# Cc19245/gaussian-splatting_CC-Comments

Hardware: AMD Instinct MI355X
Metric: train iters/sec (fwd+bwd rasterize) @1980x1080, 1M Gaussians (higher is better)
Workload: dtype f32; 1 GPU; C3: 1000000 Gaussians, SH deg 3, 1980x1080, mu=-5.0, seed 0; P=1000000, parallelism=single view

## Files before the change

gaussian-splatting_cc-comments_amd/csrc/api.hip:

```cpp
#include <stdarg.h>
#include <stdio.h>
#include <string.h>

#include <atomic>
#include <cmath>
#include <mutex>
#include <string>
#include <vector>

#include "gsr_internal.h"
#include "../../include/gsr_aa.h"
#include "../../include/gsr_contrib.h"
#include "../../include/gsr_features.h"
#include "../../include/gsr_distortion.h"
#include "../../include/gsr_median.h"
#include "../../include/gsr_normals.h"
#include "../../include/gsr_loss_ext.h"
#include "../../include/gsr_bilagrid.h"
#include "../../include/gsr_mcmc.h"
#include "../../include/gsr_densify.h"
#include "../../include/gsr_filter3d.h"
#include "../../include/gsr_knn.h"
#include "../../include/gsr_rigidity.h"

// ... 170 lines not shown
	o->col_table = off;      off = gsr_align_up(off + gsr_tilebin_col_table_bytes(n));
	o->rshape = off;         off = gsr_align_up(off + n * 8);
	o->total = off;
	return GSR_OK;
}

extern "C" int gsr_image_layout_of(int W, int H, gsr_image_layout* o)
{
	if (W < 0 || H < 0 || !o) return gsr_fail(GSR_ERR_INVALID_ARGUMENT, "gsr_image_layout_of: bad arguments");
	const size_t N = (size_t)W * H, T = (size_t)gsr_grid_x(W) * gsr_grid_y(H);
	size_t off = 0;
	o->final_C = off;          off = gsr_align_up(off + 3 * N * 4);
	o->final_T = off;          off = gsr_align_up(off + N * 4);
	o->n_contrib = off;        off = gsr_align_up(off + N * 4);
	o->ranges = off;           off = gsr_align_up(off + T * 8);
	o->tile_max_contrib = off; off = gsr_align_up(off + T * 4);
	{
		const size_t extra_f = 3 * (size_t)gsr_tile_order_max_split((int)T), extra_b = gsr_tile_order_max_segments((int)T);
		o->tile_order = off;   off = gsr_align_up(off + (T + (extra_f > extra_b ? extra_f : extra_b) + 1) * 4);
	}
	o->total = off;
	return GSR_OK;
}

extern "C" int gsr_binning_layout_of(int P, int64_t R, int W, int H, gsr_binning_layout* o)
{
	(void)P;
	if (R < 0 || W < 0 || H < 0 || !o) return gsr_fail(GSR_ERR_INVALID_ARGUMENT, "gsr_binning_layout_of: bad arguments");
	const size_t n = (size_t)R;
	size_t off = 0;
	o->point_list = off;     off = gsr_align_up(off + n * 4);
	o->point_list_alt = off; off = gsr_align_up(off + n * 4);
	o->tile_keys = off;      off = gsr_align_up(off + n * 4);
	o->tile_keys_alt = off;  off = gsr_align_up(off + n * 4);
	{
		const size_t a = gsr_radix_table_bytes(n), b = gsr_tilebin_row_table_bytes(n);
		o->sort_table = off; off = gsr_align_up(off + (a > b ? a : b));
	}
	o->checkpoints = off;    off = gsr_align_up(off + gsr_checkpoint_records(R) * 256 * sizeof(float4));
	o->total = off;
	o->tile_key_bytes = (size_t)gsr_tile_key_bytes(gsr_grid_x(W) * gsr_grid_y(H), n);
	o->column_pairs = gsr_tilebin_applies(W, H) ? 1 : 0;
	return GSR_OK;
}

extern "C" size_t gsr_geometry_bytes(int P)
{
	gsr_geometry_layout l;
	return gsr_geometry_layout_of(P, &l) == GSR_OK ? l.total : 0;
}
extern "C" size_t gsr_image_bytes(int W, int H)
{
	gsr_image_layout l;
	return gsr_image_layout_of(W, H, &l) == GSR_OK ? l.total : 0;
}
extern "C" size_t gsr_binning_bytes(int P, int64_t R, int W, int H)
{
	gsr_binning_layout l;
	return gsr_binning_layout_of(P, R, W, H, &l) == GSR_OK ? l.total : 0;
}
extern "C" size_t gsr_backward_scratch_bytes(int P, int64_t R)
{
	(void)P;
	if (R < 0) return 0;
	return gsr_align_up((size_t)R * sizeof(GsrGradSlot));
}
// ... 164 lines not shown
	g.sorted_block_sums = (uint32_t*)(b + l.scan_temp);
	g.block_tiles = (uint32_t*)(b + l.scan_temp + gsr_align_up(((size_t)P + GSR_PREPROCESS_BLOCK - 1) / GSR_PREPROCESS_BLOCK * 4));
	g.sort_table = (void*)(b + l.sort_table);
	g.col_table = (void*)(b + l.col_table);
	g.rshape = (uint2*)(b + l.rshape);
	return g;
}

GsrImage gsr_image_view(void* blob, int W, int H)
{
	gsr_image_layout l;
	gsr_image_layout_of(W, H, &l);
	char* b = (char*)blob;
	GsrImage im;
	im.final_C = (float*)(b + l.final_C);
	im.final_T = (float*)(b + l.final_T);
	im.n_contrib = (uint32_t*)(b + l.n_contrib);
	im.ranges = (uint2*)(b + l.ranges);
	im.tile_max_contrib = (uint32_t*)(b + l.tile_max_contrib);
	im.tile_order = (uint32_t*)(b + l.tile_order);
	return im;
}

GsrBinning gsr_binning_view(void* blob, int P, int64_t R, int W, int H)
{
	gsr_binning_layout l;
	gsr_binning_layout_of(P, R, W, H, &l);
	char* b = (char*)blob;
	GsrBinning bn;
	bn.point_list = (uint32_t*)(b + l.point_list);
	bn.point_list_alt = (uint32_t*)(b + l.point_list_alt);
	bn.tile_keys = (uint32_t*)(b + l.tile_keys);
	bn.tile_keys_alt = (uint32_t*)(b + l.tile_keys_alt);
	bn.sort_table = (void*)(b + l.sort_table);
	bn.checkpoints = (float4*)(b + l.checkpoints);
	return bn;
}

extern "C" uint32_t gsr_get_higher_msb(uint32_t n)
{
	uint32_t msb = sizeof(n) * 4;
	uint32_t step = msb;
	while (step > 1) {
		step /= 2;
		if (n >> msb) msb += step; else msb -= step;
	}
	if (n >> msb) msb++;
	return msb;
}

struct GsrThreadDevice {
	hipStream_t aux_stream = nullptr;
	hipEvent_t aux_fork = nullptr, aux_join = nullptr;
	uint32_t* status_host = nullptr;
	hipEvent_t status_event = nullptr;
	hipStream_t copy_stream = nullptr;
	hipEvent_t copy_fork = nullptr;
};
struct GsrThreadState { GsrThreadDevice dev[GSR_MAX_DEVICES]; };
static thread_local GsrThreadState g_thread;

extern "C" int gsr_thread_release(void)
{
	g_err[0] = 0;
	int rc = GSR_OK;
	for (int d = 0; d < GSR_MAX_DEVICES; d++) {
// ... 1338 lines not shown
```

gaussian-splatting_cc-comments_amd/csrc/gsr_internal.h:

```cpp
#pragma once
#include <hip/hip_runtime.h>
#include <hip/hip_ext.h>
#include <stddef.h>
#include <stdint.h>

#include <type_traits>

#include "../../include/gsr.h"
#include "../../include/gsr_aux.h"
#include "../../include/gsr_cam.h"
#include "../../include/gsr_absgrad.h"
#include "../../include/gsr_camera_model.h"
#include "../../include/gsr_cam_cm.h"
#include "gsr_device.h"

#define GSR_PREPROCESS_BLOCK 256
#define GSR_COUNT_PARTS 64
#define GSR_STATUS_NEGMIN (4 + GSR_COUNT_PARTS)
#define GSR_STATUS_MAX (4 + 2 * GSR_COUNT_PARTS)
#define GSR_STATUS_WORDS (4 + 3 * GSR_COUNT_PARTS)

#ifndef GSR_SLOT_COOP
#define GSR_SLOT_COOP 30
#endif
// ... 15 lines not shown
	uint8_t* clamped;
	float* sh_ddir;
	uint32_t* status;

	uint32_t* sorted_block_sums;
	uint32_t* block_tiles;
	void* sort_table;
	void* col_table;
};

#ifndef GSR_CKPT_STRIDE
#define GSR_CKPT_STRIDE 512
#endif
#ifndef GSR_SPLIT_MIN_LIST
#define GSR_SPLIT_MIN_LIST 640
#endif
#define GSR_CKPT_MAX_SEGMENTS 15
static inline size_t gsr_checkpoint_records(int64_t R) { return (size_t)(R / GSR_CKPT_STRIDE) + 2; }

struct GsrImage {
	float* final_C;
	float* final_T;
	uint32_t* n_contrib;
	uint2* ranges;
	uint32_t* tile_max_contrib;
	uint32_t* tile_order;
};

struct GsrBinning {
	uint32_t* point_list;
	uint32_t* point_list_alt;
	uint32_t* tile_keys;
	uint32_t* tile_keys_alt;
	void* sort_table;
	float4* checkpoints;
};

struct GsrAuxBlend {
	float* out_depth;
	float* out_alpha;
	float* ckpt_depth;
	float* final_D;
	const float* dL_ddepth;
	const float* dL_dalpha;
};

GsrGeometry gsr_geometry_view(void* blob, int P);
GsrImage gsr_image_view(void* blob, int W, int H);
GsrBinning gsr_binning_view(void* blob, int P, int64_t R, int W, int H);

struct GsrFrame {
	int P, W, H;
	int64_t R;
	GsrGeometry g;
	GsrImage img;
	GsrBinning bin;
	GsrGradSlot* slots;
	uint8_t* slot_valid;
	hipStream_t s;
	int debug;
	bool cull;
};

struct GsrCamTarget {
	float* rows;
	float* dL_dviewmatrix;
// ... 255 lines not shown
```

gaussian-splatting_cc-comments_amd/csrc/render_backward.hip:

```cpp
#include "render_common.h"
#include <type_traits>

#define GSR_BWD_NV 9
#ifndef GSR_BWD_BAND_LAST
#define GSR_BWD_BAND_LAST 1
#endif
#define GSR_BWD_FLUSH 4
typedef float v2f __attribute__((ext_vector_type(2)));

GSR_TILE_CLOCK_BUFFER(gsr_backward_tile_clock, gsr_debug_tile_clock_backward)

__device__ __forceinline__ float gsr_add_halves(v2f a)
{
	float r;
	asm("v_add_f32_e32 %0, %1, %2" : "=v"(r) : "v"(a.x), "v"(a.y));
	return r;
}

template <int M> struct gsr_half;
template <> struct gsr_half<3> {
	typedef v2f type;
	static __device__ __forceinline__ v2f get(const v2f& a) { return a; }
	static __device__ __forceinline__ void set(v2f& d, v2f s) { d = s; }
	static __device__ __forceinline__ v2f select(bool h0, bool h1, v2f a) { return v2f{h0 ? a.x : 0.f, h1 ? a.y : 0.f}; }
};
template <> struct gsr_half<1> {
	typedef float type;
	static __device__ __forceinline__ float get(const v2f& a) { return a.x; }
	static __device__ __forceinline__ void set(v2f& d, float s) { d.x = s; }
	static __device__ __forceinline__ float select(bool h0, bool, float a) { return h0 ? a : 0.f; }
};
template <> struct gsr_half<2> {
	typedef float type;
	static __device__ __forceinline__ float get(const v2f& a) { return a.y; }
	static __device__ __forceinline__ void set(v2f& d, float s) { d.y = s; }
	static __device__ __forceinline__ float select(bool, bool h1, float a) { return h1 ? a : 0.f; }
};
__device__ __forceinline__ float gsr_fma(float a, float b, float c) { return __builtin_fmaf(a, b, c); }
__device__ __forceinline__ v2f gsr_fma(v2f a, v2f b, v2f c) { return __builtin_elementwise_fma(a, b, c); }
__device__ __forceinline__ float gsr_exp2(float a) { return __builtin_amdgcn_exp2f(a); }
__device__ __forceinline__ v2f gsr_exp2(v2f a) { return v2f{__builtin_amdgcn_exp2f(a.x), __builtin_amdgcn_exp2f(a.y)}; }
__device__ __forceinline__ float gsr_rcp(float a) { return __builtin_amdgcn_rcpf(a); }
__device__ __forceinline__ v2f gsr_rcp(v2f a) { return v2f{__builtin_amdgcn_rcpf(a.x), __builtin_amdgcn_rcpf(a.y)}; }
__device__ __forceinline__ float gsr_min99(float a) { return fminf(0.99f, a); }
__device__ __forceinline__ v2f gsr_min99(v2f a) { return v2f{fminf(0.99f, a.x), fminf(0.99f, a.y)}; }
__device__ __forceinline__ float gsr_lo(float a) { return a; }
__device__ __forceinline__ float gsr_lo(v2f a) { return a.x; }
__device__ __forceinline__ float gsr_hi(float a) { return a; }
__device__ __forceinline__ float gsr_hi(v2f a) { return a.y; }
__device__ __forceinline__ float gsr_abs_sum(float a) { return __builtin_fabsf(a); }
__device__ __forceinline__ float gsr_abs_sum(v2f a) { return __builtin_fabsf(a.x) + __builtin_fabsf(a.y); }

template <bool AUX, bool ABS>
__global__ void __launch_bounds__(64 * GSR_WAVES_PER_WG) __attribute__((amdgpu_waves_per_eu((AUX && ABS) ? 3 : 4, 4))) gsr_render_backward_wave_kernel(
	int W, int H, int gx, int nslots, const uint2* __restrict__ ranges, const uint32_t* __restrict__ point_list,
	const GsrSplat* __restrict__ splat, const float4* __restrict__ checkpoints, const float* __restrict__ final_C, const uint32_t* __restrict__ slot_base, const float* __restrict__ bg,
	const float* __restrict__ final_Ts, const uint32_t* __restrict__ n_contrib, const uint32_t* __restrict__ tile_max_contrib,
	const uint32_t* __restrict__ tile_order, const float* __restrict__ dL_dpixels, GsrGradSlot* __restrict__ slots,
	uint8_t* __restrict__ slot_valid, int cull, GsrAuxBlend aux)
{
	__shared__ float4 s_rec[GSR_WAVES_PER_WG][AUX ? 6 : 5][64];
	__shared__ uint32_t s_bands[GSR_WAVES_PER_WG][64];
	__shared__ float s_red[GSR_WAVES_PER_WG][64 * 9 + 8];
	__shared__ __attribute__((aligned(16))) float s_pend[GSR_WAVES_PER_WG][(AUX || ABS) ? 4 : GSR_BWD_FLUSH * 128];
	constexpr bool ONE_BAND = !(AUX || ABS);
	const int wave = threadIdx.x >> 6, lane = threadIdx.x & 63;
	const int slot_id = blockIdx.x * GSR_WAVES_PER_WG + wave;
	if (slot_id >= nslots) return;
	GSR_TILE_CLOCK_START();
	GSR_TILE_STAT(unsigned long long st_staged = 0; unsigned long long st_pairs = 0; unsigned long long st_pairs_hit = 0; unsigned long long st_reductions = 0; unsigned long long st_lanes_hit = 0;
	              unsigned long long st_one_mask = 0; unsigned long long st_one_last = 0;)
	const uint32_t entry = __builtin_amdgcn_readfirstlane(tile_order[slot_id]);
	if (entry == 0xFFFFFFFFu) return;
	const int tile = (int)(entry & 0x0FFFFFFFu);
	const int seg1 = (int)(entry >> 28);
	float4(*rec)[64] = s_rec[wave];
	uint32_t* recb = s_bands[wave];

	const int tx = tile % gx, ty = tile / gx;
	const int px = tx * GSR_TILE_X + (lane & 15);
	const int py0 = ty * GSR_TILE_Y + (lane >> 4);
	const v2f pfx2 = {(float)px, (float)px};
	const float x0f = (float)(tx * GSR_TILE_X), y0f = (float)(ty * GSR_TILE_Y);

	const uint2 range = ranges[tile];
	const int n = (int)min(range.y - range.x, tile_max_contrib[tile]);
	int seg_a = 0, top = n;
	if (seg1) {
		const int coarse = (int)__builtin_amdgcn_readfirstlane(tile_order[nslots]);
		const int nblk = (n + GSR_CKPT_STRIDE - 1) / GSR_CKPT_STRIDE, m = (nblk + GSR_CKPT_MAX_SEGMENTS - 1) / GSR_CKPT_MAX_SEGMENTS * coarse;
		seg_a = (seg1 - 1) * m * GSR_CKPT_STRIDE;
		top = min(n, seg1 * m * GSR_CKPT_STRIDE);
	}
	const int nw = top - seg_a;
	const uint32_t* plist = point_list + range.x;
	const size_t plane = (size_t)H * W;
	const float bg0 = bg[0], bg1 = bg[1], bg2 = bg[2];
	const float ddelx_dx = 0.5f * W, ddely_dy = 0.5f * H;

	v2f T[2], tfb[2];
	v2f ac0[2], ac1[2], ac2[2];
	v2f dp0[2], dp1[2], dp2[2];
	v2f dpD[2], acD[2];
	int last_contributor[GSR_PIX_PER_LANE];
	v2f pfy[2];
#pragma unroll
	for (int k = 0; k < GSR_PIX_PER_LANE; k++) {
		const int py = py0 + 4 * k;
		const bool inside = px < W && py < H;
		const uint32_t pix_id = inside ? (uint32_t)(W * py + px) : 0u;
		const float Tf = inside ? final_Ts[pix_id] : 0.f;
		const float d0 = inside ? dL_dpixels[pix_id] : 0.f;
		const float d1 = inside ? dL_dpixels[plane + pix_id] : 0.f;
		const float d2 = inside ? dL_dpixels[2 * plane + pix_id] : 0.f;
		last_contributor[k] = inside ? (int)n_contrib[pix_id] : 0;
		T[k >> 1][k & 1] = Tf;
		dp0[k >> 1][k & 1] = d0; dp1[k >> 1][k & 1] = d1; dp2[k >> 1][k & 1] = d2;
		if (AUX) {
			const float dD = (inside && aux.dL_ddepth) ? aux.dL_ddepth[pix_id] : 0.f;
			const float dA = (inside && aux.dL_dalpha) ? aux.dL_dalpha[pix_id] : 0.f;
			dpD[k >> 1][k & 1] = dD;
			tfb[k >> 1][k & 1] = -Tf * ((bg0 * d0 + bg1 * d1 + bg2 * d2) - dA);
		} else {
			tfb[k >> 1][k & 1] = -Tf * (bg0 * d0 + bg1 * d1 + bg2 * d2);
		}
		pfy[k >> 1][k & 1] = (float)py;
	}
#pragma unroll
	for (int p = 0; p < 2; p++) {
		ac0[p] = ac1[p] = ac2[p] = v2f{0.f, 0.f};
		if (AUX) acD[p] = v2f{0.f, 0.f};
	}
	if (top < n) {
		const float4* ck = checkpoints + ((size_t)(range.x + (uint32_t)top) / GSR_CKPT_STRIDE) * 256 + lane;
#pragma unroll
		for (int k = 0; k < GSR_PIX_PER_LANE; k++) {
			const int py = py0 + 4 * k;
			const bool inside = px < W && py < H;
			const uint32_t pix_id = inside ? (uint32_t)(W * py + px) : 0u;
			if (inside && last_contributor[k] > top) {
				const float4 c = ck[64 * k];
				const float inv = 1.0f / c.x;
				T[k >> 1][k & 1] = c.x;
				ac0[k >> 1][k & 1] = (final_C[pix_id] - c.y) * inv;
				ac1[k >> 1][k & 1] = (final_C[plane + pix_id] - c.z) * inv;
				ac2[k >> 1][k & 1] = (final_C[2 * plane + pix_id] - c.w) * inv;
				if (AUX) acD[k >> 1][k & 1] = (aux.final_D[pix_id] - aux.ckpt_depth[((size_t)(range.x + (uint32_t)top) / GSR_CKPT_STRIDE) * 256 + lane + 64 * k]) * inv;
			}
		}
	}
	int band_last[GSR_PIX_PER_LANE];
#pragma unroll
	for (int k = 0; k < GSR_PIX_PER_LANE; k++) {
		int m = last_contributor[k];
#pragma unroll
		for (int off = 32; off > 0; off >>= 1) m = max(m, __shfl_xor(m, off, 64));
		band_last[k] = __builtin_amdgcn_readfirstlane(m);
	}

	float4 ra = make_float4(0, 0, 0, 0), rb = ra, rc = ra;
	uint32_t sbase = 0u;
	if (lane < nw) {
		const uint32_t id = plist[top - 1 - lane];
		const float4* p = reinterpret_cast<const float4*>(splat + id);
		ra = p[0]; rb = p[1]; rc = p[2];
		sbase = slot_base[id];
	}
	uint32_t id_next = (64 + lane < nw) ? plist[top - 1 - (64 + lane)] : 0u;
	const int out_index = lane >> 3;
	float* const red_w = s_red[wave] + lane * 9;
	const float* const red_r = s_red[wave] + (lane & 7) * 9 + (lane >> 3);
	constexpr int red_step = 72;
	const float out_scale = (out_index >= 2 && out_index <= 4) ? -0.5f : 1.0f;
	const float k01 = out_index == 0 ? -ddelx_dx : -ddely_dy;
	const int f_inst = (lane >> 3) & 3, f_val = lane & 7;
	float* const pend_w = s_pend[wave] + lane;
	const float* const pend_r = s_pend[wave] + f_inst * 128 + (lane >> 5) * 64 + f_val * 8;
	const float f_scale = (f_val >= 2 && f_val <= 4) ? -0.5f : 1.0f;
	const float f_k01 = f_val == 0 ? -ddelx_dx : -ddely_dy;
	const bool f_word = lane < 32 || f_val == 0;
	int npend = 0;
	uint32_t pend_j = 0u;

	for (int base = 0; base < nw; base += 64) {
		const uint32_t reach = (base + lane < nw) ? (cull ? gsr_tile_band_mask(ra.x, ra.y, ra.z, ra.w, rb.x, rb.y, x0f, y0f) : 0xFu) : 0u;
		const int position = top - 1 - (base + lane);
		uint32_t live = 0u;
#pragma unroll
		for (int k = 0; k < GSR_PIX_PER_LANE; k++) live |= position < band_last[k] ? 1u << k : 0u;
		if (!(cull && GSR_BWD_BAND_LAST)) live = ((live & 3u) ? 3u : 0u) | ((live & 12u) ? 12u : 0u);
		const uint32_t bands = reach & live;
		const bool keep = cull ? bands != 0u : reach != 0u;
		const unsigned long long mask = __builtin_amdgcn_ballot_w64(keep);
		const int cnt = __popcll(mask);
		GSR_TILE_STAT(st_staged += (unsigned)cnt;)
		if (keep) {
			const int pos = gsr_mbcnt(mask);
			const uint32_t rmin = __float_as_uint(rb.z), rwh = __float_as_uint(rb.w);
			const uint32_t slot = sbase + ((uint32_t)ty - (rmin >> 16)) * (rwh & 0xffffu) + ((uint32_t)tx - (rmin & 0xffffu));
			rec[0][pos] = make_float4(ra.x, ra.x, ra.y, ra.y);
			rec[1][pos] = make_float4(-0.5f * ra.z, -0.5f * ra.z, ra.w, ra.w);
			rec[2][pos] = make_float4(-0.5f * rb.x, -0.5f * rb.x, rb.y, rb.y);
			rec[3][pos] = make_float4(rc.x, rc.x, rc.y, rc.y);
			rec[4][pos] = make_float4(rc.z, rc.z, __int_as_float(position), __uint_as_float(slot));
			if (AUX) rec[5][pos] = make_float4(rc.w, rc.w, 0.f, 0.f);
			recb[pos] = bands | (reach << 4);
		}
		if (base + 64 + lane < nw) {
			const float4* p = reinterpret_cast<const float4*>(splat + id_next);
			ra = p[0]; rb = p[1]; rc = p[2];
			sbase = slot_base[id_next];
		}
		id_next = (base + 128 + lane < nw) ? plist[top - 1 - (base + 128 + lane)] : 0u;
		__builtin_amdgcn_wave_barrier();

#pragma clang loop unroll(disable)
		for (int j = 0; j < cnt; j++) {
			const float4 R0 = rec[0][j], R1 = rec[1][j], R2 = rec[2][j], R3 = rec[3][j], R4 = rec[4][j];
			const int contributor = __builtin_amdgcn_readfirstlane(__float_as_int(R4.z));
			const uint32_t bands = __builtin_amdgcn_readfirstlane(recb[j]);
			const v2f X = {R0.x, R0.y}, Y = {R0.z, R0.w}, CA = {R1.x, R1.y}, CB = {R1.z, R1.w}, CC = {R2.x, R2.y}, OP = {R2.z, R2.w};
			const v2f C0 = {R3.x, R3.y}, C1 = {R3.z, R3.w}, C2 = {R4.x, R4.y};
			v2f V = {0.f, 0.f};
			if (AUX) { const float4 R5 = rec[5][j]; V = v2f{R5.x, R5.y}; }
			const v2f dx = X - pfx2;
			const v2f ax2 = (CA * dx) * dx, bdx = CB * dx;
			v2f CBh = {0.f, 0.f};
			float absx = 0.f, absy = 0.f;
			if constexpr (ABS) CBh = -0.5f * CB;
			v2f acc[GSR_BWD_NV + 1];
#pragma unroll
			for (int i = 0; i < GSR_BWD_NV + 1; i++) acc[i] = v2f{-0.f, -0.f};
			unsigned long long any = 0ull;
			auto pair = [&](auto pc, auto mc) {
				constexpr int p = decltype(pc)::value, M = decltype(mc)::value;
				typedef gsr_half<M> Hf;
				typedef typename Hf::type V_t;
				const V_t dxh = Hf::get(dx);
				const V_t dy = Hf::get(Y) - Hf::get(pfy[p]);
				const V_t power = (Hf::get(ax2) + (Hf::get(CC) * dy) * dy) - Hf::get(bdx) * dy;
				const V_t pl = power * 1.44269504088896340736f;
				const V_t G = gsr_exp2(pl);
				const V_t og = Hf::get(OP) * G;
				const V_t araw = gsr_min99(og);
				bool hit0 = false, hit1 = false;
				unsigned long long hits = 0ull;
// ... 112 lines not shown
					pend_w[npend * 128] = tcol;
					pend_w[npend * 128 + 64] = v[8];
					pend_j |= (uint32_t)j << (8 * npend);
					npend++;
				}
			}
			if (!(AUX || ABS) && (npend == GSR_BWD_FLUSH || (npend != 0 && j == cnt - 1))) {
				__builtin_amdgcn_wave_barrier();
				const float4 q0 = *reinterpret_cast<const float4*>(pend_r), q1 = *reinterpret_cast<const float4*>(pend_r + 4);
				const uint32_t jf = (pend_j >> (8 * f_inst)) & 0xFFu;
				const float* const rj = reinterpret_cast<const float*>(&rec[0][jf]);
				const float ca = rj[4 * 64], cb = rj[4 * 64 + 2], cc = rj[8 * 64];
				const uint32_t slot = __float_as_uint(rj[16 * 64 + 3]);
				asm volatile("" ::"v"(q0.x), "v"(q1.x), "v"(ca), "v"(cb), "v"(cc), "v"(slot));
				const float t = ((q0.x + q0.y) + (q0.z + q0.w)) + ((q1.x + q1.y) + (q1.z + q1.w));
				const float t9 = gsr_sum8(t);
				const float other = gsr_dpp_mov<0xB1, 0xF, 0xF, true>(t);
				const float r01 = f_k01 * __builtin_fmaf(-2.0f, (f_val == 0 ? ca : cc) * t, cb * other);
				const float r = f_val < 2 ? r01 : f_scale * t;
				if (f_inst < npend) {
					if (f_word) reinterpret_cast<float*>(slots + slot)[lane < 32 ? f_val : 8] = lane < 32 ? r : t9;
					if (lane >= 32 && f_val == 0) slot_valid[slot] = 1;
				}
				npend = 0;
				pend_j = 0u;
				__builtin_amdgcn_wave_barrier();
			}
		}
		__builtin_amdgcn_wave_barrier();
	}
	GSR_TILE_CLOCK_STOP(gsr_backward_tile_clock, slot_id, lane, st_staged | (st_pairs << 20) | (st_pairs_hit << 42), st_reductions | (st_lanes_hit << 24), st_one_mask | (st_one_last << 32));
}

void gsr_launch_render_backward(const GsrFrame& f, const float* bg, const float* dL_dpix, hipEvent_t t_start, hipEvent_t t_stop,
                                const GsrAuxBlend* aux, bool absgrad)
{
	const GsrImage& img = f.img;
	const int W = f.W, H = f.H, gx = gsr_grid_x(W), gy = gsr_grid_y(H);
	const int ntiles = gx * gy;
	const int nslots = ntiles + (int)gsr_tile_order_max_segments(ntiles);
	const int nwg = (nslots + GSR_WAVES_PER_WG - 1) / GSR_WAVES_PER_WG;
	gsr_variant(false, aux ? GSR_AUX_DEPTH : 0, absgrad, [&](auto, auto AUX, auto ABS) {
		gsr_launch(gsr_render_backward_wave_kernel<AUX() != 0, ABS()>, dim3(nwg), dim3(64 * GSR_WAVES_PER_WG), 0, f.s, t_start, t_stop, W, H, gx, nslots,
		           img.ranges, f.bin.point_list, f.g.splat, f.bin.checkpoints, img.final_C, f.g.slot_base, bg, img.final_T, img.n_contrib,
		           img.tile_max_contrib, img.tile_order, dL_dpix, f.slots, f.slot_valid, f.cull ? 1 : 0, aux ? *aux : GsrAuxBlend{});
	});
}
```

gaussian-splatting_cc-comments_amd/csrc/render_forward.hip:

```cpp
#include "render_common.h"

#ifndef GSR_FWD_DONE_STRIDE
#define GSR_FWD_DONE_STRIDE 16
#endif
#ifndef GSR_FWD_AUX_WAVES
#define GSR_FWD_AUX_WAVES 5
#endif

GSR_TILE_CLOCK_BUFFER(gsr_forward_tile_clock, gsr_debug_tile_clock_forward)

template <bool AUX>
__global__ void __launch_bounds__(64 * GSR_WAVES_PER_WG) __attribute__((amdgpu_waves_per_eu(AUX ? GSR_FWD_AUX_WAVES : 6, AUX ? GSR_FWD_AUX_WAVES : 6)))
gsr_render_forward_wave_kernel(
	int W, int H, int gx, int nslots, const uint2* __restrict__ ranges, const uint32_t* __restrict__ point_list,
	const GsrSplat* __restrict__ splat, float4* __restrict__ checkpoints, float* __restrict__ final_C, const float* __restrict__ bg, float* __restrict__ final_T,
	uint32_t* __restrict__ n_contrib, uint32_t* __restrict__ tile_max_contrib, const uint32_t* __restrict__ tile_order,
	float* __restrict__ out_color, int cull, GsrAuxBlend aux)
{
	__shared__ float4 s_rec[GSR_WAVES_PER_WG][3][64];
	const int wave = threadIdx.x >> 6, lane = threadIdx.x & 63;
	const int slot_id = blockIdx.x * GSR_WAVES_PER_WG + wave;
	if (slot_id >= nslots) return;
	GSR_TILE_CLOCK_START();
	const uint32_t entry = __builtin_amdgcn_readfirstlane(tile_order ? tile_order[slot_id] : (uint32_t)slot_id);
	if (entry == 0xFFFFFFFFu) return;
	const int tile = (int)(entry & 0x0FFFFFFFu);
	const int only = (int)(entry >> 28);
	float4(*rec)[64] = s_rec[wave];

	const int tx = tile % gx, ty = tile / gx;
	const int px = tx * GSR_TILE_X + (lane & 15);
	const int py0 = ty * GSR_TILE_Y + (lane >> 4);
	float pfx = (float)px;
	asm volatile("" : "+v"(pfx));
	const float x0f = (float)(tx * GSR_TILE_X), y0f = (float)(ty * GSR_TILE_Y);

	const uint2 range = ranges[tile];
	const int n = (int)(range.y - range.x);
	const uint32_t* plist = point_list + range.x;
	const bool heavy = n >= 2 * GSR_CKPT_STRIDE;
	bool walked_deep = false;

	float Tout[GSR_PIX_PER_LANE], C0[GSR_PIX_PER_LANE], C1[GSR_PIX_PER_LANE], C2[GSR_PIX_PER_LANE];
	float Dacc[GSR_PIX_PER_LANE];
	float pfy[GSR_PIX_PER_LANE];
	uint32_t last[GSR_PIX_PER_LANE];
	unsigned long long alive[GSR_PIX_PER_LANE];
#pragma unroll
	for (int k = 0; k < GSR_PIX_PER_LANE; k++) {
		const int py = py0 + 4 * k;
		pfy[k] = (float)py;
		asm volatile("" : "+v"(pfy[k]));
		Tout[k] = 1.0f;
		alive[k] = (only == 0 || only == k + 1) ? __builtin_amdgcn_ballot_w64(px < W && py < H) : 0ull;
		C0[k] = C1[k] = C2[k] = 0.f;
		if (AUX) Dacc[k] = 0.f;
		last[k] = 0u;
	}

	GSR_TILE_STAT(unsigned long long st_staged = 0ull; unsigned long long st_bands = 0ull; unsigned long long st_hits = 0ull;)
	float4 ra = make_float4(0, 0, 0, 0), rb = ra, rc = ra;
	if (lane < n) {
		const uint32_t id = plist[lane];
		const float4* p = reinterpret_cast<const float4*>(splat + id);
		ra = p[0]; rb = p[1]; rc = p[2];
	}
	uint32_t id_next = (64 + lane < n) ? plist[64 + lane] : 0u;

	for (int base = 0; base < n; base += 64) {
		if ((alive[0] | alive[1] | alive[2] | alive[3]) == 0ull) break;
		if (heavy && base != 0 && (base & (GSR_CKPT_STRIDE - 1)) == 0) {
			walked_deep = true;
			float4* ck = checkpoints + ((size_t)(range.x + (uint32_t)base) / GSR_CKPT_STRIDE) * 256 + lane;
#pragma unroll
			for (int k = 0; k < GSR_PIX_PER_LANE; k++)
				if (only == 0 || only == k + 1) ck[64 * k] = make_float4(Tout[k], C0[k], C1[k], C2[k]);
			if (AUX) {
				float* ckd = aux.ckpt_depth + ((size_t)(range.x + (uint32_t)base) / GSR_CKPT_STRIDE) * 256 + lane;
#pragma unroll
				for (int k = 0; k < GSR_PIX_PER_LANE; k++)
					if (only == 0 || only == k + 1) ckd[64 * k] = Dacc[k];
			}
		}
		const uint32_t bands = (base + lane < n) ? (cull ? gsr_tile_band_mask(ra.x, ra.y, ra.z, ra.w, rb.x, rb.y, x0f, y0f) : 0xFu) : 0u;
		const bool keep = bands != 0u;
		const unsigned long long mask = __builtin_amdgcn_ballot_w64(keep);
		const int cnt = __popcll(mask);
		GSR_TILE_STAT(st_staged += (unsigned long long)cnt;)
		if (keep) {
			const int pos = gsr_mbcnt(mask);
			rec[0][pos] = make_float4(ra.x, ra.y, -0.5f * ra.z, ra.w);
			rec[1][pos] = make_float4(-0.5f * rb.x, rb.y, rc.x, rc.y);
			rec[2][pos] = make_float4(rc.z, __uint_as_float((uint32_t)(base + lane + 1)), __uint_as_float(bands), AUX ? rc.w : 0.f);
		}
		if (base + 64 + lane < n) {
			const float4* p = reinterpret_cast<const float4*>(splat + id_next);
			ra = p[0]; rb = p[1]; rc = p[2];
		}
		id_next = (base + 128 + lane < n) ? plist[base + 128 + lane] : 0u;
		__builtin_amdgcn_wave_barrier();

		for (int j0 = 0; j0 < cnt; j0 += GSR_FWD_DONE_STRIDE) {
		const uint32_t open_bands = __builtin_amdgcn_readfirstlane((alive[0] ? 1u : 0u) | (alive[1] ? 2u : 0u) | (alive[2] ? 4u : 0u) | (alive[3] ? 8u : 0u));
		if (open_bands == 0u) break;
		const int j1 = min(cnt, j0 + GSR_FWD_DONE_STRIDE);
		for (int j = j0; j < j1; j++) {
			const float4 A = rec[0][j];
			const float4 B = rec[1][j];
			const float4 Cc = rec[2][j];
			const uint32_t contributor = __float_as_uint(Cc.y);
			uint32_t bands = __builtin_amdgcn_readfirstlane(__float_as_uint(Cc.z)) & open_bands;
			asm volatile("" : "+s"(bands));
			const float dx = A.x - pfx;
			const float ax2 = __fmul_rn(__fmul_rn(A.z, dx), dx), bdx = __fmul_rn(A.w, dx);
#pragma unroll
			for (int k = 0; k < GSR_PIX_PER_LANE; k++) {
				if (!(bands & (1u << k))) continue;
// ... 31 lines not shown
			n_contrib[pix_id] = last[k];
			out_color[pix_id] = C0[k] + Tout[k] * bg0;
			out_color[plane + pix_id] = C1[k] + Tout[k] * bg1;
			out_color[2 * plane + pix_id] = C2[k] + Tout[k] * bg2;
			if (walked_deep) { final_C[pix_id] = C0[k]; final_C[plane + pix_id] = C1[k]; final_C[2 * plane + pix_id] = C2[k]; }
			if (AUX) {
				aux.out_depth[pix_id] = Dacc[k];
				aux.out_alpha[pix_id] = 1.0f - Tout[k];
				if (walked_deep) aux.final_D[pix_id] = Dacc[k];
			}
			m = max(m, last[k]);
		}
	}
#pragma unroll
	for (int off = 32; off > 0; off >>= 1) m = max(m, (uint32_t)__shfl_down(m, off, 64));
	if (lane == 0) {
		if (only) atomicMax(&tile_max_contrib[tile], m);
		else tile_max_contrib[tile] = m;
	}
	GSR_TILE_CLOCK_STOP(gsr_forward_tile_clock, slot_id, lane, (unsigned long long)entry,
	                    (st_staged & 0xFFFFFull) | ((st_bands & 0x3FFFFFull) << 20) | ((st_hits & 0x3FFFFFull) << 42), 0ull);
}

void gsr_launch_render_forward(const GsrFrame& f, const float* bg, float* out_color, bool ordered, const GsrAuxBlend* aux)
{
	const GsrImage& img = f.img;
	const int W = f.W, H = f.H, gx = gsr_grid_x(W), gy = gsr_grid_y(H);
	const int ntiles = gx * gy;
	const int nslots = ntiles + (ordered ? 3 * (int)gsr_tile_order_max_split(ntiles) : 0);
	const int nwg = (nslots + GSR_WAVES_PER_WG - 1) / GSR_WAVES_PER_WG;
	gsr_variant(false, aux ? GSR_AUX_DEPTH : 0, false, [&](auto, auto AUX, auto) {
		gsr_launch(gsr_render_forward_wave_kernel<AUX() != 0>, dim3(nwg), dim3(64 * GSR_WAVES_PER_WG), 0, f.s, nullptr, nullptr, W, H, gx, nslots,
		           img.ranges, f.bin.point_list, f.g.splat, f.bin.checkpoints, img.final_C, bg, img.final_T, img.n_contrib, img.tile_max_contrib,
		           ordered ? img.tile_order : nullptr, out_color, f.cull ? 1 : 0, aux ? *aux : GsrAuxBlend{});
	});
}
```

gaussian-splatting_cc-comments_amd/diff_gaussian_rasterization/_C.py:

```python
import ctypes
import math
import os
from typing import NamedTuple, Optional

import torch

_HERE = os.path.dirname(os.path.abspath(__file__))
_LIB_PATH = os.path.join(os.path.dirname(_HERE), "libgsr_hip.so")
_lib = None

_vp = ctypes.c_void_p
_i = ctypes.c_int
_i64 = ctypes.c_int64
_f = ctypes.c_float
_sz = ctypes.c_size_t


class GeometryLayout(ctypes.Structure):
    _fields_ = [(n, _sz) for n in ("splat", "depth_keys", "depth_keys_alt", "perm", "perm_alt", "tiles_touched", "rect",
                                   "slot_base", "clamped", "sh_ddir", "status", "scan_temp", "sort_table", "col_table", "rshape", "total")]


class ImageLayout(ctypes.Structure):
    _fields_ = [(n, _sz) for n in ("final_C", "final_T", "n_contrib", "ranges", "tile_max_contrib", "tile_order", "total")]


class BinningLayout(ctypes.Structure):
    _fields_ = [(n, _sz) for n in ("point_list", "point_list_alt", "tile_keys", "tile_keys_alt", "sort_table",
                                   "checkpoints", "total", "tile_key_bytes", "column_pairs")]


class KernelTime(ctypes.Structure):
    _fields_ = [("name", ctypes.c_char_p), ("ms", _f)]


class BackwardArgs(ctypes.Structure):
    _fields_ = ([("P", _i), ("D", _i), ("M", _i), ("num_rendered", _i64), ("width", _i), ("height", _i), ("leaf", _i)] +
                [(n, _vp) for n in ("background", "means3D", "shs", "shs_rest", "colors_precomp", "scales")] +
                [("scale_modifier", _f)] +
                [(n, _vp) for n in ("rotations", "cov3D_precomp", "viewmatrix", "projmatrix", "cam_pos")] +
                [("tan_fovx", _f), ("tan_fovy", _f)] +
                [(n, _vp) for n in ("radii", "geometry", "binning", "image", "scratch", "dL_dpix", "dL_dmean2D", "dL_dconic",
                                    "dL_dopacity", "dL_dcolor", "dL_dmean3D", "dL_dcov3D", "dL_dsh", "dL_dsh_rest", "dL_dscale",
                                    "dL_drot", "stat_xyz_gradient_accum", "stat_denom", "stat_max_radii2D", "stream")] +
                [("debug", _i)])


AUX_MODES = {"depth": 1, "invdepth": 2}


class AuxArgs(ctypes.Structure):
    _fields_ = [("mode", _i), ("out_depth", _vp), ("out_alpha", _vp), ("dL_ddepth", _vp), ("dL_dalpha", _vp), ("scratch", _vp)]


class CamArgs(ctypes.Structure):
    _fields_ = [("dL_dviewmatrix", _vp), ("dL_dprojmatrix", _vp), ("dL_dcampos", _vp), ("scratch", _vp)]


class CamCmArgs(ctypes.Structure):
    _fields_ = [("dL_dviewmatrix", _vp), ("dL_dintrinsics", _vp), ("dL_dcampos", _vp), ("scratch", _vp)]


class AbsgradArgs(ctypes.Structure):
    _fields_ = [("abs_dL_dmean2D", _vp), ("stat_abs_gradient_accum", _vp)]


class CameraModelArgs(ctypes.Structure):
    _fields_ = [("model", _i), ("fx", _f), ("fy", _f), ("cx", _f), ("cy", _f)]


CAMERA_MODELS = {"pinhole": 0, "fisheye": 1}


class CameraModel(NamedTuple):
    model: str
    fx: float
    fy: float
    cx: float
    cy: float

    @classmethod
    def from_tensor(cls, model, intrinsics):
        if not isinstance(intrinsics, torch.Tensor) or tuple(intrinsics.shape) != (4,):
            raise ValueError(f"intrinsics must be a tensor of shape (4,) holding (fx, fy, cx, cy), got {intrinsics!r}")
        return camera_model((model, *(float(v) for v in intrinsics.detach().to(torch.float32).cpu().tolist())))


class AuxLayout(ctypes.Structure):
    _fields_ = [(n, _sz) for n in ("ckpt_depth", "final_D", "total")]


DEBUG_SYNC, DEBUG_NO_CULL, DEBUG_SERIAL, DEBUG_NO_SPLIT, DEBUG_TILE_SORT, DEBUG_RADIX_DEPTH, DEBUG_NO_TRIM = 1, 2, 4, 8, 16, 32, 64
DEBUG_MEDIAN_FULL_WALK = 128


def _dbg(debug):
    return int(debug) if (isinstance(debug, int) and not isinstance(debug, bool)) else int(bool(debug))


def library_path():
    return _LIB_PATH


def use_library(path):
    global _LIB_PATH
    if _lib is not None:
        raise RuntimeError("use_library() must be called before the library is first loaded")
    _LIB_PATH = os.path.abspath(path)


def lib():
    global _lib
    if _lib is not None:
        return _lib
    if not os.path.exists(_LIB_PATH):
        raise RuntimeError(
            f"{_LIB_PATH} not found: build it with `python -c 'import __graft_entry__ as g; g.build()'` "
            "(hipcc --offload-arch=gfx950).  There is no CPU fallback for the rasterizer.")
    L = ctypes.CDLL(_LIB_PATH)
    L.gsr_last_error.restype = ctypes.c_char_p
    L.gsr_version.restype = ctypes.c_char_p
    L.gsr_geometry_bytes.restype = _sz
    L.gsr_geometry_bytes.argtypes = [_i]
    L.gsr_image_bytes.restype = _sz
    L.gsr_image_bytes.argtypes = [_i, _i]
    L.gsr_binning_bytes.restype = _sz
# ... 929 lines not shown
```

include/gsr.h:

```cpp
#ifndef GSR_H_INCLUDED
#define GSR_H_INCLUDED

#include <stddef.h>
#include <stdint.h>

#ifdef __cplusplus
extern "C" {
#endif

typedef enum {
	GSR_OK = 0,
	GSR_ERR_INVALID_ARGUMENT = -1,
	GSR_ERR_HIP = -2,
	GSR_ERR_PREFILTERED = -3,
	GSR_ERR_BUFFER_TOO_SMALL = -4
} gsr_status;

#define GSR_DEBUG_SYNC    1
#define GSR_DEBUG_NO_CULL 2
#define GSR_DEBUG_SERIAL  4
#define GSR_DEBUG_TILE_SORT 16
#define GSR_DEBUG_RADIX_DEPTH 32
#define GSR_DEBUG_NO_TRIM 64
#define GSR_DEBUG_NO_SPLIT 8

const char* gsr_last_error(void);

const char* gsr_version(void);

int gsr_thread_release(void);

size_t gsr_geometry_bytes(int P);
size_t gsr_image_bytes(int width, int height);
size_t gsr_binning_bytes(int P, int64_t num_rendered, int width, int height);
size_t gsr_backward_scratch_bytes(int P, int64_t num_rendered);

typedef struct {
	size_t splat;
	size_t depth_keys;
	size_t depth_keys_alt;
	size_t perm;
	size_t perm_alt;
	size_t tiles_touched;
	size_t rect;
	size_t slot_base;
	size_t clamped;
	size_t sh_ddir;
	size_t status;
	size_t scan_temp;
	size_t sort_table;
	size_t col_table;
	size_t rshape;
	size_t total;
} gsr_geometry_layout;

typedef struct {
	size_t final_C;
	size_t final_T;
	size_t n_contrib;
	size_t ranges;
	size_t tile_max_contrib;
	size_t tile_order;
	size_t total;
} gsr_image_layout;

typedef struct {
	size_t point_list;
	size_t point_list_alt;
	size_t tile_keys;
	size_t tile_keys_alt;
	size_t sort_table;
	size_t checkpoints;
	size_t total;
	size_t tile_key_bytes;
	size_t column_pairs;
} gsr_binning_layout;

int gsr_geometry_layout_of(int P, gsr_geometry_layout* out);
int gsr_image_layout_of(int width, int height, gsr_image_layout* out);
int gsr_binning_layout_of(int P, int64_t num_rendered, int width, int height, gsr_binning_layout* out);

int gsr_forward_preprocess(
	int P, int D, int M,
	int width, int height,
	const float* means3D,
	const float* shs,
	const float* colors_precomp,
	const float* opacities,
	const float* scales,
	float scale_modifier,
	const float* rotations,
	const float* cov3D_precomp,
	const float* viewmatrix,
	const float* projmatrix,
	const float* cam_pos,
	float tan_fovx, float tan_fovy,
	int prefiltered,
	int* radii,
	void* geometry,
	int64_t* num_rendered_host,
	void* stream, int debug);

int gsr_forward_render(
	int P, int64_t num_rendered,
	int width, int height,
	const float* background,
	const int* radii,
	void* geometry, void* binning, void* image,
// ... 114 lines not shown
```

Before: 1013 it/s.

## Cache per-entry tile band masks from forward for reuse in backward blend

The forward blend kernel now stores each sorted entry's tile band mask into a byte array carved out of the binning buffer. The backward kernel reads these masks instead of recomputing the band test, and skips loading splat data for entries whose mask is zero. The old recompute path stays available behind a debug flag. This adds a byte store in forward and a byte load in backward, and places the mask array inside the tile_keys region, assuming it is dead by then.

```diff
diff --git a/gaussian-splatting_cc-comments_amd/csrc/api.hip b/gaussian-splatting_cc-comments_amd/csrc/api.hip
--- a/gaussian-splatting_cc-comments_amd/csrc/api.hip
+++ b/gaussian-splatting_cc-comments_amd/csrc/api.hip
@@ -226,6 +226,7 @@
 	o->point_list = off;     off = gsr_align_up(off + n * 4);
 	o->point_list_alt = off; off = gsr_align_up(off + n * 4);
 	o->tile_keys = off;      off = gsr_align_up(off + n * 4);
+	o->band_masks = off + gsr_align_up(n, 4);
 	o->tile_keys_alt = off;  off = gsr_align_up(off + n * 4);
 	{
 		const size_t a = gsr_radix_table_bytes(n), b = gsr_tilebin_row_table_bytes(n);
@@ -456,6 +457,7 @@
 	bn.point_list_alt = (uint32_t*)(b + l.point_list_alt);
 	bn.tile_keys = (uint32_t*)(b + l.tile_keys);
 	bn.tile_keys_alt = (uint32_t*)(b + l.tile_keys_alt);
+	bn.band_masks = (uint8_t*)(b + l.band_masks);
 	bn.sort_table = (void*)(b + l.sort_table);
 	bn.checkpoints = (float4*)(b + l.checkpoints);
 	return bn;
diff --git a/gaussian-splatting_cc-comments_amd/csrc/gsr_internal.h b/gaussian-splatting_cc-comments_amd/csrc/gsr_internal.h
--- a/gaussian-splatting_cc-comments_amd/csrc/gsr_internal.h
+++ b/gaussian-splatting_cc-comments_amd/csrc/gsr_internal.h
@@ -71,6 +71,7 @@
 	uint32_t* point_list_alt;
 	uint32_t* tile_keys;
 	uint32_t* tile_keys_alt;
+	uint8_t* band_masks;
 	void* sort_table;
 	float4* checkpoints;
 };
diff --git a/gaussian-splatting_cc-comments_amd/csrc/render_backward.hip b/gaussian-splatting_cc-comments_amd/csrc/render_backward.hip
--- a/gaussian-splatting_cc-comments_amd/csrc/render_backward.hip
+++ b/gaussian-splatting_cc-comments_amd/csrc/render_backward.hip
@@ -51,10 +51,10 @@
 __device__ __forceinline__ float gsr_abs_sum(float a) { return __builtin_fabsf(a); }
 __device__ __forceinline__ float gsr_abs_sum(v2f a) { return __builtin_fabsf(a.x) + __builtin_fabsf(a.y); }
 
-template <bool AUX, bool ABS>
-__global__ void __launch_bounds__(64 * GSR_WAVES_PER_WG) __attribute__((amdgpu_waves_per_eu((AUX && ABS) ? 3 : 4, 4))) gsr_render_backward_wave_kernel(
+template <bool AUX, bool ABS, bool RECOMPUTE>
+__device__ __forceinline__ void gsr_render_backward_wave(
 	int W, int H, int gx, int nslots, const uint2* __restrict__ ranges, const uint32_t* __restrict__ point_list,
-	const GsrSplat* __restrict__ splat, const float4* __restrict__ checkpoints, const float* __restrict__ final_C, const uint32_t* __restrict__ slot_base, const float* __restrict__ bg,
+	const uint8_t* __restrict__ band_masks, const GsrSplat* __restrict__ splat, const float4* __restrict__ checkpoints, const float* __restrict__ final_C, const uint32_t* __restrict__ slot_base, const float* __restrict__ bg,
 	const float* __restrict__ final_Ts, const uint32_t* __restrict__ n_contrib, const uint32_t* __restrict__ tile_max_contrib,
 	const uint32_t* __restrict__ tile_order, const float* __restrict__ dL_dpixels, GsrGradSlot* __restrict__ slots,
 	uint8_t* __restrict__ slot_valid, int cull, GsrAuxBlend aux)
@@ -94,6 +94,7 @@
 	}
 	const int nw = top - seg_a;
 	const uint32_t* plist = point_list + range.x;
+	const uint8_t* pmask = band_masks + range.x;
 	const size_t plane = (size_t)H * W;
 	const float bg0 = bg[0], bg1 = bg[1], bg2 = bg[2];
 	const float ddelx_dx = 0.5f * W, ddely_dy = 0.5f * H;
@@ -160,13 +161,19 @@
 
 	float4 ra = make_float4(0, 0, 0, 0), rb = ra, rc = ra;
 	uint32_t sbase = 0u;
-	if (lane < nw) {
+	auto mask_at = [&](int q) -> uint32_t {
+		if (RECOMPUTE || q >= nw) return 0u;
+		return cull ? (uint32_t)pmask[top - 1 - q] : 0xFu;
+	};
+	uint32_t m_cur = mask_at(lane);
+	if (RECOMPUTE ? lane < nw : m_cur != 0u) {
 		const uint32_t id = plist[top - 1 - lane];
 		const float4* p = reinterpret_cast<const float4*>(splat + id);
 		ra = p[0]; rb = p[1]; rc = p[2];
 		sbase = slot_base[id];
 	}
 	uint32_t id_next = (64 + lane < nw) ? plist[top - 1 - (64 + lane)] : 0u;
+	uint32_t m_next = mask_at(64 + lane);
 	const int out_index = lane >> 3;
 	float* const red_w = s_red[wave] + lane * 9;
 	const float* const red_r = s_red[wave] + (lane & 7) * 9 + (lane >> 3);
@@ -183,7 +190,8 @@
 	uint32_t pend_j = 0u;
 
 	for (int base = 0; base < nw; base += 64) {
-		const uint32_t reach = (base + lane < nw) ? (cull ? gsr_tile_band_mask(ra.x, ra.y, ra.z, ra.w, rb.x, rb.y, x0f, y0f) : 0xFu) : 0u;
+		uint32_t reach = m_cur;
+		if constexpr (RECOMPUTE) reach = (base + lane < nw) ? (cull ? gsr_tile_band_mask(ra.x, ra.y, ra.z, ra.w, rb.x, rb.y, x0f, y0f) : 0xFu) : 0u;
 		const int position = top - 1 - (base + lane);
 		uint32_t live = 0u;
 #pragma unroll
@@ -206,12 +214,14 @@
 			if (AUX) rec[5][pos] = make_float4(rc.w, rc.w, 0.f, 0.f);
 			recb[pos] = bands | (reach << 4);
 		}
-		if (base + 64 + lane < nw) {
+		if (RECOMPUTE ? base + 64 + lane < nw : m_next != 0u) {
 			const float4* p = reinterpret_cast<const float4*>(splat + id_next);
 			ra = p[0]; rb = p[1]; rc = p[2];
 			sbase = slot_base[id_next];
 		}
+		m_cur = m_next;
 		id_next = (base + 128 + lane < nw) ? plist[top - 1 - (base + 128 + lane)] : 0u;
+		m_next = mask_at(base + 128 + lane);
 		__builtin_amdgcn_wave_barrier();
 
 #pragma clang loop unroll(disable)
@@ -390,6 +400,23 @@
 	GSR_TILE_CLOCK_STOP(gsr_backward_tile_clock, slot_id, lane, st_staged | (st_pairs << 20) | (st_pairs_hit << 42), st_reductions | (st_lanes_hit << 24), st_one_mask | (st_one_last << 32));
 }
 
+#define GSR_BWD_KERNEL(name, RECOMPUTE)                                                                                                        \
+	template <bool AUX, bool ABS>                                                                                                              \
+	__global__ void __launch_bounds__(64 * GSR_WAVES_PER_WG) __attribute__((amdgpu_waves_per_eu((AUX && ABS) ? 3 : 4, 4))) name(                \
+		int W, int H, int gx, int nslots, const uint2* __restrict__ ranges, const uint32_t* __restrict__ point_list,                           \
+		const uint8_t* __restrict__ band_masks, const GsrSplat* __restrict__ splat, const float4* __restrict__ checkpoints,                    \
+		const float* __restrict__ final_C, const uint32_t* __restrict__ slot_base, const float* __restrict__ bg,                               \
+		const float* __restrict__ final_Ts, const uint32_t* __restrict__ n_contrib, const uint32_t* __restrict__ tile_max_contrib,             \
+		const uint32_t* __restrict__ tile_order, const float* __restrict__ dL_dpixels, GsrGradSlot* __restrict__ slots,                        \
+		uint8_t* __restrict__ slot_valid, int cull, GsrAuxBlend aux)                                                                           \
+	{                                                                                                                                          \
+		gsr_render_backward_wave<AUX, ABS, RECOMPUTE>(W, H, gx, nslots, ranges, point_list, band_masks, splat, checkpoints, final_C, slot_base, bg, \
+		                                              final_Ts, n_contrib, tile_max_contrib, tile_order, dL_dpixels, slots, slot_valid, cull, aux); \
+	}
+GSR_BWD_KERNEL(gsr_render_backward_wave_kernel, false)
+GSR_BWD_KERNEL(gsr_render_backward_recompute_kernel, true)
+#undef GSR_BWD_KERNEL
+
 void gsr_launch_render_backward(const GsrFrame& f, const float* bg, const float* dL_dpix, hipEvent_t t_start, hipEvent_t t_stop,
                                 const GsrAuxBlend* aux, bool absgrad)
 {
@@ -398,9 +425,11 @@
 	const int ntiles = gx * gy;
 	const int nslots = ntiles + (int)gsr_tile_order_max_segments(ntiles);
 	const int nwg = (nslots + GSR_WAVES_PER_WG - 1) / GSR_WAVES_PER_WG;
-	gsr_variant(false, aux ? GSR_AUX_DEPTH : 0, absgrad, [&](auto, auto AUX, auto ABS) {
-		gsr_launch(gsr_render_backward_wave_kernel<AUX() != 0, ABS()>, dim3(nwg), dim3(64 * GSR_WAVES_PER_WG), 0, f.s, t_start, t_stop, W, H, gx, nslots,
-		           img.ranges, f.bin.point_list, f.g.splat, f.bin.checkpoints, img.final_C, f.g.slot_base, bg, img.final_T, img.n_contrib,
+	gsr_variant((f.debug & GSR_DEBUG_RECOMPUTE_BANDS) != 0, aux ? GSR_AUX_DEPTH : 0, absgrad, [&](auto RECOMPUTE, auto AUX, auto ABS) {
+		auto kernel = gsr_render_backward_wave_kernel<AUX() != 0, ABS()>;
+		if (RECOMPUTE()) kernel = gsr_render_backward_recompute_kernel<AUX() != 0, ABS()>;
+		gsr_launch(kernel, dim3(nwg), dim3(64 * GSR_WAVES_PER_WG), 0, f.s, t_start, t_stop, W, H, gx, nslots,
+		           img.ranges, f.bin.point_list, f.bin.band_masks, f.g.splat, f.bin.checkpoints, img.final_C, f.g.slot_base, bg, img.final_T, img.n_contrib,
 		           img.tile_max_contrib, img.tile_order, dL_dpix, f.slots, f.slot_valid, f.cull ? 1 : 0, aux ? *aux : GsrAuxBlend{});
 	});
 }
diff --git a/gaussian-splatting_cc-comments_amd/csrc/render_forward.hip b/gaussian-splatting_cc-comments_amd/csrc/render_forward.hip
--- a/gaussian-splatting_cc-comments_amd/csrc/render_forward.hip
+++ b/gaussian-splatting_cc-comments_amd/csrc/render_forward.hip
@@ -15,7 +15,7 @@
 	int W, int H, int gx, int nslots, const uint2* __restrict__ ranges, const uint32_t* __restrict__ point_list,
 	const GsrSplat* __restrict__ splat, float4* __restrict__ checkpoints, float* __restrict__ final_C, const float* __restrict__ bg, float* __restrict__ final_T,
 	uint32_t* __restrict__ n_contrib, uint32_t* __restrict__ tile_max_contrib, const uint32_t* __restrict__ tile_order,
-	float* __restrict__ out_color, int cull, GsrAuxBlend aux)
+	float* __restrict__ out_color, uint8_t* __restrict__ band_masks, int cull, GsrAuxBlend aux)
 {
 	__shared__ float4 s_rec[GSR_WAVES_PER_WG][3][64];
 	const int wave = threadIdx.x >> 6, lane = threadIdx.x & 63;
@@ -38,6 +38,7 @@
 	const uint2 range = ranges[tile];
 	const int n = (int)(range.y - range.x);
 	const uint32_t* plist = point_list + range.x;
+	uint8_t* const pmask = band_masks + range.x;
 	const bool heavy = n >= 2 * GSR_CKPT_STRIDE;
 	bool walked_deep = false;
 
@@ -83,6 +84,7 @@
 			}
 		}
 		const uint32_t bands = (base + lane < n) ? (cull ? gsr_tile_band_mask(ra.x, ra.y, ra.z, ra.w, rb.x, rb.y, x0f, y0f) : 0xFu) : 0u;
+		if (base + lane < n) pmask[base + lane] = (uint8_t)bands;
 		const bool keep = bands != 0u;
 		const unsigned long long mask = __builtin_amdgcn_ballot_w64(keep);
 		const int cnt = __popcll(mask);
@@ -180,6 +182,6 @@
 	gsr_variant(false, aux ? GSR_AUX_DEPTH : 0, false, [&](auto, auto AUX, auto) {
 		gsr_launch(gsr_render_forward_wave_kernel<AUX() != 0>, dim3(nwg), dim3(64 * GSR_WAVES_PER_WG), 0, f.s, nullptr, nullptr, W, H, gx, nslots,
 		           img.ranges, f.bin.point_list, f.g.splat, f.bin.checkpoints, img.final_C, bg, img.final_T, img.n_contrib, img.tile_max_contrib,
-		           ordered ? img.tile_order : nullptr, out_color, f.cull ? 1 : 0, aux ? *aux : GsrAuxBlend{});
+		           ordered ? img.tile_order : nullptr, out_color, f.bin.band_masks, f.cull ? 1 : 0, aux ? *aux : GsrAuxBlend{});
 	});
 }
diff --git a/gaussian-splatting_cc-comments_amd/diff_gaussian_rasterization/_C.py b/gaussian-splatting_cc-comments_amd/diff_gaussian_rasterization/_C.py
--- a/gaussian-splatting_cc-comments_amd/diff_gaussian_rasterization/_C.py
+++ b/gaussian-splatting_cc-comments_amd/diff_gaussian_rasterization/_C.py
@@ -27,7 +27,7 @@
 
 class BinningLayout(ctypes.Structure):
     _fields_ = [(n, _sz) for n in ("point_list", "point_list_alt", "tile_keys", "tile_keys_alt", "sort_table",
-                                   "checkpoints", "total", "tile_key_bytes", "column_pairs")]
+                                   "checkpoints", "total", "tile_key_bytes", "column_pairs", "band_masks")]
 
 
 class KernelTime(ctypes.Structure):
@@ -92,6 +92,7 @@
 
 DEBUG_SYNC, DEBUG_NO_CULL, DEBUG_SERIAL, DEBUG_NO_SPLIT, DEBUG_TILE_SORT, DEBUG_RADIX_DEPTH, DEBUG_NO_TRIM = 1, 2, 4, 8, 16, 32, 64
 DEBUG_MEDIAN_FULL_WALK = 128
+DEBUG_RECOMPUTE_BANDS = 256
 
 
 def _dbg(debug):
diff --git a/include/gsr.h b/include/gsr.h
--- a/include/gsr.h
+++ b/include/gsr.h
@@ -23,6 +23,7 @@
 #define GSR_DEBUG_RADIX_DEPTH 32
 #define GSR_DEBUG_NO_TRIM 64
 #define GSR_DEBUG_NO_SPLIT 8
+#define GSR_DEBUG_RECOMPUTE_BANDS 256
 
 const char* gsr_last_error(void);
 
@@ -74,6 +75,7 @@
 	size_t total;
 	size_t tile_key_bytes;
 	size_t column_pairs;
+	size_t band_masks;
 } gsr_binning_layout;
 
 int gsr_geometry_layout_of(int P, gsr_geometry_layout* out);
```

New measurement: 1023 it/s, median of 6. 1.1% higher.
